# pierrepaleo/sift_pyocl

Hardware: AMD Instinct MI355X
Metric: SiftPlan.keypoints throughput, 4096x4096 fp32 (Mpix/s; keypoints/s in keypoints_per_s) (higher is better)
Workload: dtype f32

## Files before the change

### sift_pyocl_amd/csrc/k_pyramid.hpp

```cpp
#pragma once
#include <hip/hip_runtime.h>
#include <type_traits>
#include <stdint.h>
#include "k_xcd.hpp"

namespace siftk {

__device__ __forceinline__ uint32_t f2ord(float f) {
    uint32_t u = __float_as_uint(f);
    return (u & 0x80000000u) ? ~u : (u | 0x80000000u);
}
__device__ __forceinline__ float ord2f(uint32_t u) {
    return __uint_as_float((u & 0x80000000u) ? (u & 0x7fffffffu) : ~u);
}

__global__ void minmax_init(uint32_t *mm) { mm[0] = 0xffffffffu; mm[1] = 0u; }

__device__ __forceinline__ void minmax_reset_next(uint32_t *reset, int reset_words, int reset_ones) {
    if (reset && blockIdx.x == 0)
        for (int i = threadIdx.x; i < reset_words; i += blockDim.x) reset[i] = (i == reset_ones) ? 0xffffffffu : 0u;
}

__global__ __launch_bounds__(1024) void minmax_kernel(const float *__restrict__ img, int64_t n, uint32_t *mm, uint32_t *reset = nullptr,
                                                      int reset_words = 0, int reset_ones = -1) {
// ... 450 lines not shown
                        }                                                                                    \
                        const int done = (kk + 1) % N;                                                       \
                        const int y = ybase_ + kk;                                                           \
                        if (y >= ys && y < yend && !((BLUR_ABL & 8) && acc[done].x != 12345.678f)) {        \
                            if (vec_store) *reinterpret_cast<f32x2 *>(optr) = acc[done];                     \
                            else { if (gxo < W) optr[0] = acc[done].x; if (gxo + 1 < W) optr[1] = acc[done].y; } \
                            if (next0 && !(y & 1) && (y >> 1) < (H >> 1) && (gxo >> 1) < (W >> 1))           \
                                next0[(size_t)(y >> 1) * (W >> 1) + (gxo >> 1)] = acc[done].x;              \
                        }                                                                                    \
                        optr += W;                                                                           \
                    }                                                                                        \
                }                                                                                            \
            }                                                                                                \
        }                                                                                                    \
    }

    auto exists = [&](int blk, int sub) { return blk < nblocks - 1 || (blk == nblocks - 1 && sub < last_subs); };
    if (role == 1) {
        prefetch(0, 0, SS::pairs(0));
        stage(sbase, SS::pairs(0));
        if (S > 1) { if (exists(0, 1 % S)) prefetch(0, 1 % S, SS::pairs(1 % S)); }
        else if (exists(1, 0)) prefetch(1, 0, SS::pairs(0));
    }
    __syncthreads();
    int g = 0;
    const int total_steps = (nblocks - 1) * S + last_subs;
    int prio_level = -1;
    auto set_prio = [&](int step) {
        if (!prio) return;
        const int q = (step * 4) / total_steps;
        if (q == prio_level) return;
        prio_level = q;
        if (q <= 0) __builtin_amdgcn_s_setprio(3);
        else if (q == 1) __builtin_amdgcn_s_setprio(2);
        else if (q == 2) __builtin_amdgcn_s_setprio(1);
        else __builtin_amdgcn_s_setprio(0);
    };
    set_prio(0);
    if (role == 0) {
        for (int blk = 0; blk < nblocks; blk++) {
#pragma unroll
            for (int sub = 0; sub < S; sub++) {
                if (blk == nblocks - 1 && sub >= last_subs) break;
                hpass(sbase + (g % 3) * BUF, SS::pairs(sub));
                __syncthreads();
                g++;
                set_prio(g);
            }
        }
        return;
    }
    for (int blk = 0; blk < nblocks; blk++) {
#pragma unroll
        for (int sub = 0; sub < S; sub++) {
            if (blk == nblocks - 1 && sub >= last_subs) break;
            if (g > 0) {
                float *prev = sbase + ((g + 2) % 3) * BUF;
                if (sub == 0) { VPASS(prev, blk - 1, S - 1) } else { VPASS(prev, blk, (sub + S - 1) % S) }
            }
            const int sub1 = (sub + 1) % S, blk1 = blk + (sub + 1) / S;
            if (exists(blk1, sub1)) {
                float *nxt = sbase + ((g + 1) % 3) * BUF;
                stage(nxt, SS::pairs(sub1));
                const int sub2 = (sub + 2) % S;
                const int blk2 = blk + (sub + 2) / S;
                if (exists(blk2, sub2)) prefetch(blk2, sub2, SS::pairs(sub2));
            }
            __syncthreads();
            g++;
            set_prio(g);
        }
    }
    {
        float *prev = sbase + ((g + 2) % 3) * BUF;
        if (last_subs >= S) { VPASS(prev, nblocks - 1, S - 1) }
        if constexpr (S > 1) { if (last_subs == 1) { VPASS(prev, nblocks - 1, 0) } }
        if constexpr (S > 2) { if (last_subs == 2) { VPASS(prev, nblocks - 1, 1) } }
        if constexpr (S > 3) { if (last_subs == 3) { VPASS(prev, nblocks - 1, 2) } }
    }
#undef VPASS
}


__global__ void blur_generic_pass(const float *__restrict__ in, float *__restrict__ out, int W, int H,
                                  const float *__restrict__ taps, int n, int vertical,
                                  const uint32_t *__restrict__ mm, int norm) {
    const int x = blockIdx.x * blockDim.x + threadIdx.x, y = blockIdx.y;
    if (x >= W || y >= H) return;
    const int c = (n & 1) ? n / 2 : n / 2 - 1;
    float mn = 0.f, range = 1.f;
    if (norm) { mn = ord2f(mm[0]); range = ord2f(mm[1]) - mn; }
    float acc = 0.f;
    for (int j = 0; j < n; j++) {
        float v;
        if (vertical) v = in[(size_t)reflect_index(y - c + j, H) * W + x];
        else v = in[(size_t)y * W + reflect_index(x - c + j, W)];
        if (norm) v = 255.0f * (v - mn) / range;
        acc = acc + v * taps[n - 1 - j];
    }
    out[(size_t)y * W + x] = acc;
}

__global__ __launch_bounds__(256) void shrink_kernel(const float *__restrict__ in, float *__restrict__ out, int LW, int SW, int SH) {
    const int x = (blockIdx.x * 64 + (threadIdx.x & 63)) * 4;
    const int y0 = (blockIdx.y * 4 + (threadIdx.x >> 6)) * 2;
    if (x >= SW) return;
    const bool vec_in = (LW & 1) == 0 && x + 3 < SW;
    const bool vec_out = (SW & 3) == 0;
#pragma unroll
    for (int r = 0; r < 2; r++) {
        const int y = y0 + r;
        if (y >= SH) break;
        const float *src = in + (size_t)(2 * y) * LW + 2 * x;
        float *dst = out + (size_t)y * SW + x;
        if (vec_in) {
            const float4 a = *reinterpret_cast<const float4 *>(src), b = *reinterpret_cast<const float4 *>(src + 4);
            if (vec_out) *reinterpret_cast<float4 *>(dst) = make_float4(a.x, a.z, b.x, b.z);
            else { dst[0] = a.x; dst[1] = a.z; dst[2] = b.x; dst[3] = b.z; }
        } else {
            for (int k = 0; k < 4 && x + k < SW; k++) dst[k] = src[2 * k];
        }
    }
}
inline dim3 shrink_grid(int SW, int SH) { return dim3((unsigned)((SW + 255) / 256), (unsigned)((SH + 7) / 8)); }

template <int DT = 0>
__global__ void normalize_kernel(const void *__restrict__ in, float *__restrict__ out, int64_t n,
                                 const uint32_t *__restrict__ mm) {
    const float mn = ord2f(mm[0]), range = ord2f(mm[1]) - mn;
    const int64_t stride = (int64_t)gridDim.x * blockDim.x;
    for (int64_t i = (int64_t)blockIdx.x * blockDim.x + threadIdx.x; i < n; i += stride)
        out[i] = 255.0f * (load_px<DT>(in, (size_t)i) - mn) / range;
}

}
```

### sift_pyocl_amd/csrc/siftmi.hip

```cpp
#include <hip/hip_runtime.h>
#include <hip/hip_ext.h>

#include <cmath>
#include <cstdarg>
#include <cstdio>
#include <cstdlib>
#include <cstring>
#include <algorithm>
#include <chrono>
#include <mutex>
#include <new>
#include <unordered_map>
#include <string>
#include <vector>

#include "../../include/siftmi.h"
#include "k_extrema.hpp"
#include "k_keypoint.hpp"
#include "k_descriptor.hpp"
#include "k_align.hpp"
#include "k_match.hpp"
#include "k_pyramid.hpp"
#include "k_tail.hpp"
#include "siftmath.hpp"

using namespace siftk;

static_assert(sizeof(siftmi_keypoint) == 144, "siftmi_keypoint must be 144 bytes");

namespace {

thread_local std::string g_err;

#ifndef SIFT_SYNC_EVENT
#define SIFT_SYNC_EVENT (hipEventDisableTiming | hipEventDisableSystemFence)
#endif
#define SIFTMI_ETAILRETRY (-100)
#define SIFTMI_EGROW (-101)
int fail(int code, const char *fmt, ...) {
    char buf[512];
    va_list ap;
    va_start(ap, fmt);
    vsnprintf(buf, sizeof buf, fmt, ap);
    va_end(ap);
    g_err = buf;
    return code;
}

#define HIPCHK(expr)                                                                           \
    do {                                                                                       \
        hipError_t e_ = (expr);                                                                \
        if (e_ != hipSuccess)                                                                  \
            return fail(e_ == hipErrorOutOfMemory ? SIFTMI_ENOMEM : SIFTMI_EDEVICE, "%s: %s", #expr, \
                        hipGetErrorString(e_));                                                \
    } while (0)

int nextpower(int n) { int p = 1; while (p < n) p <<= 1; return p; }

int gaussian_taps(float sigma, int size, float *out) {
    if (size < 1 || size > 1024) return fail(SIFTMI_EINVAL, "gaussian size %d out of range", size);
    int P = nextpower(size);
    if (P < 2) P = 2;
    std::vector<float> g((size_t)P, 0.0f), sum((size_t)P, 0.0f);
    const float norm = sqrtf(2.0f * SM_PI_F);
    for (int i = 0; i < size; i++) {
        const float x = ((float)i - ((float)size - 1.0f) / 2.0f) / sigma;
        const float y = siftmath::expf_(-x * x / 2.0f);
        g[(size_t)i] = y / sigma / norm;
        sum[(size_t)i] = g[(size_t)i];
    }
    for (int stride = 512; stride >= 2; stride >>= 1)
        if (size > stride)
            for (int i = 0; i < stride && i + stride < P; i++) sum[(size_t)i] += sum[(size_t)(i + stride)];
    sum[0] += sum[1];
    for (int i = 0; i < size; i++) out[i] = g[(size_t)i] / sum[0];
    return SIFTMI_OK;
}

int kernel_size(double sigma) {
    int size = (int)std::ceil(2.0 * 4.0 * sigma + 1.0);
    if (size % 2 == 0) size += 1;
    return size;
}

struct Taps { int n = 0; float t[64] = {0}; float *dev = nullptr; };

#define SIFT_LDS_PAD_MAX 65536

struct Options {
    int fused_convert = 1;
    int overlap = 1;
    int march = 1;
    int march_wgs = 0;
    int xcd_map = 1;
    int march_prio = 1;
    int ori_blocks = 4096, ori_pad = 0;
    int desc_blocks = 960, desc_pad = 0;
    int desc_small_blocks = 576;
    int desc_dense_blocks = 960;
    int desc_stream = 0;
    int maps = 2, maps_density = 200;
    int maps_blocks = 8192;
    int mm_blocks = 256;
    int mm_threads = 1024;
    int desc_team = 2048;
    int fork = 2;
    int split = 0;
    int early_chain = 2;
    int desc_early_blocks = 704;
    int fused_refine = 1;
    int fused_shrink = 1;
    int ori_team = 1024;
    int desc_dynamic = 1;
    int tail_pixels = SIFT_TAIL_MAX_PIXELS;
    int tail = 1;
    int ext_rows = 0;
    int ext_strips = 2000;
    int ori_small_blocks = 608;
    int spin = 1;
    int host_timing = 0;
    int tail_fault = 0;
};
const Options g_default_options{};

struct Event { std::string label; hipEvent_t a = nullptr, b = nullptr; bool is_blur = false; double pixels = 0; int octave = -1; int launches = 1; };

size_t dtype_size(int dt) {
    switch (dt) {
        case SIFTMI_F32: return 4; case SIFTMI_U8: return 1; case SIFTMI_U16: return 2; case SIFTMI_U32: return 4;
        case SIFTMI_U64: return 8; case SIFTMI_I32: return 4; case SIFTMI_I64: return 8; case SIFTMI_F64: return 8;
        case SIFTMI_RGB8: return 3;
    }
    return 0;
}

}

struct GroupLists {
    float4 *kp = nullptr;  int *kp_aux = nullptr;  int64_t cap_kp = 0;
    float4 *okp = nullptr; int *oaux = nullptr;    int64_t cap_out = 0;
    float4 *cand = nullptr; int64_t cap_cand = 0;
};

struct siftmi_plan {
    void *chain = nullptr;
    int device = 0;
    hipStream_t stream = nullptr;
    int H = 0, W = 0, dtype = 0;
    siftmi_params par{};
    Options opt;
    int profile = 0;
    int n_oct = 0;
    std::vector<int> ow, oh;
    int64_t kpsize = 0;
    int64_t bytes = 0;
    float *planes = nullptr;
    std::vector<size_t> oct_off;
    float *tmp = nullptr;
    float *tmp_later = nullptr;
    float *tmp_below = nullptr;
    hipStream_t stream2 = nullptr;
    hipStream_t stream3 = nullptr;
    int64_t acc_calls = 0, acc_b0_launches = 0;
    double acc_total_ms = 0, acc_b0_ms = 0, acc_b0_pixels = 0;
    hipEvent_t ev_early = nullptr;
    hipEvent_t ev_p3 = nullptr;
    std::vector<hipEvent_t> ev_pyr;
    bool overlap = true;
    float *plane(int o, int s) const { return planes + oct_off[(size_t)o] + (size_t)s * (size_t)ow[(size_t)o] * (size_t)oh[(size_t)o]; }
    void *raw = nullptr;
    int raw_dtype = -1;
    Counters *cnt_pair = nullptr;
    int cnt_parity = 0;
    hipStream_t fin = nullptr;
    int last_group0 = 0;
// ... 25 lines not shown
    int64_t cap_rec = 0;
    bool in_flight = false;
    bool records_cut = false;
    int64_t grows = 0;
    int64_t tail_timeouts = 0;
    KpRecord *host_out = nullptr;
    int host_cap = 0;
    bool desc_rows = true;
    Taps taps[6];
    bool have_init = false;
    std::vector<Event> events;
    size_t n_events = 0;
    hipEvent_t ev_first = nullptr, ev_last[3] = {nullptr, nullptr, nullptr};
    float last_min = 0, last_max = 0;
    int64_t last_count = 0;
    int last_overflow = 0;
    std::vector<void *> allocs;

    template <class T> int alloc(T **p, size_t nbytes) {
        void *q = nullptr;
        hipError_t e = hipMalloc(&q, nbytes ? nbytes : 16);
        if (e != hipSuccess) return fail(SIFTMI_ENOMEM, "hipMalloc(%zu bytes): %s", nbytes, hipGetErrorString(e));
        allocs.push_back(q);
        bytes += (int64_t)nbytes;
        *p = (T *)q;
        return SIFTMI_OK;
    }
    template <class T> int regrow(T **p, size_t old_bytes, size_t new_bytes) {
        void *q = nullptr;
        hipError_t e = hipMalloc(&q, new_bytes ? new_bytes : 16);
        if (e != hipSuccess) return fail(SIFTMI_ENOMEM, "hipMalloc(%zu bytes): %s", new_bytes, hipGetErrorString(e));
        if (*p) { (void)hipFree(*p); bytes -= (int64_t)old_bytes; }
        bytes += (int64_t)new_bytes;
        *p = (T *)q;
        return SIFTMI_OK;
    }
};

namespace {

int compute_schedule(siftmi_plan *p) {
    const double init_sigma = p->par.init_sigma;
    p->have_init = false;
    p->desc_rows = (int)(1.414 * 3.0 * init_sigma * std::pow(2.0, 1.5) * 2.5 + 0.5) + 2 <= SIFT_DESC_MAXRAD;
    const double cur_sigma = p->par.double_im_size ? 1.0 : 0.5;
    if (init_sigma > cur_sigma) {
        const double s = std::sqrt(init_sigma * init_sigma - cur_sigma * cur_sigma);
        p->taps[5].n = kernel_size(s);
        if (p->taps[5].n > 64) return fail(SIFTMI_EINVAL, "init_sigma %g needs %d taps (> 64)", init_sigma, p->taps[5].n);
        int rc = gaussian_taps((float)s, p->taps[5].n, p->taps[5].t);
        if (rc) return rc;
        p->have_init = true;
    }
    const double ratio = std::pow(2.0, 1.0 / 3.0);
    double prev = init_sigma;
    for (int s = 0; s < 5; s++) {
        const double inc = prev * std::sqrt(ratio * ratio - 1.0);
        p->taps[s].n = kernel_size(inc);
        if (p->taps[s].n > 64) return fail(SIFTMI_EINVAL, "sigma %g needs %d taps (> 64)", inc, p->taps[s].n);
        int rc = gaussian_taps((float)inc, p->taps[s].n, p->taps[s].t);
        if (rc) return rc;
        prev *= ratio;
    }
    for (int s = 0; s < 6; s++) {
        if (!p->taps[s].dev) { int rc = p->alloc(&p->taps[s].dev, 64 * sizeof(float)); if (rc) return rc; }
        HIPCHK(hipMemcpy(p->taps[s].dev, p->taps[s].t, 64 * sizeof(float), hipMemcpyHostToDevice));
    }
    return SIFTMI_OK;
}

template <typename K, typename... A>
inline void launch_ev(hipEvent_t stop, K kernel, dim3 grid, dim3 block, size_t lds, hipStream_t st, A... args) {
    if (stop) hipExtLaunchKernelGGL(kernel, grid, block, (uint32_t)lds, st, nullptr, stop, 0u, args...);
    else hipLaunchKernelGGL(kernel, grid, block, lds, st, args...);
}

template <int N, bool NORM, int DT, int TX, int TY, int VR>
void launch_blur_geom(hipStream_t st, const void *in, float *out, int W, int H, const TapsArg<N> &ta, const uint32_t *mm, float *half, hipEvent_t stop = nullptr) {
    using G = BlurGeom<N, TX, TY>;
    dim3 grid((unsigned)((W + TX - 1) / TX), (unsigned)((H + TY - 1) / TY));
    launch_ev(stop, blur_hv_kernel<N, NORM, DT, TX, TY, VR>, grid, dim3(256), (size_t)G::LDS_BYTES, st, in, out, W, H, ta, mm, half);
}

template <int N, bool NORM, int DT = 0>
void launch_blur_t(const Options &opt, hipStream_t st, const void *in, float *out, int W, int H, const float *taps, const uint32_t *mm, float *half = nullptr, hipEvent_t stop = nullptr) {
    TapsArg<N> ta;
    for (int i = 0; i < N; i++) ta.t[i] = taps[i];
    (void)opt;
    launch_blur_geom<N, NORM, DT, 32, 16, 4>(st, in, out, W, H, ta, mm, half, stop);
}

template <int N, bool NORM, int S, int DT = 0>
void launch_team(const Options &opt, hipStream_t st, const void *in, float *out, int W, int H, const float *taps, const uint32_t *mm, int wgs, float *half, hipEvent_t stop) {
    using G = March2Geom<N, 128, S>;
    using SS = SubSplit<N, S>;
    TapsArg<N> ta;
    for (int i = 0; i < N; i++) ta.t[i] = taps[i];
    if (opt.march_wgs > 0) wgs = opt.march_wgs;
    const int gx = (W + G::TX - 1) / G::TX;
    int gy = wgs / gx;
    if (gy < 1) gy = 1;
    if (gy > H) gy = H;
    int rows_out = (H + gy - 1) / gy;
    if (rows_out < 2 * N + 1) rows_out = 2 * N + 1;
    gy = (H + rows_out - 1) / rows_out;
    auto covered = [](int b, int m) { int r = b * N; for (int q = 0; q < m; q++) r += SS::rows(q); return r; };
    const int need = rows_out + N - 1;
    const int b = need / N;
    int m = 0;
    while (covered(b, m) < need) m++;
    const int nblocks = b + (m > 0 ? 1 : 0), last_subs = m > 0 ? m : S;
    dim3 grid((unsigned)gx, (unsigned)gy);
    const int prio = (opt.march_prio == 2 || (opt.march_prio == 1 && gx * gy >= 704)) ? 1 : 0;
    launch_ev(stop, blur_team_kernel<N, NORM, S, DT>, grid, dim3(256), (size_t)3 * G::LDS_BYTES, st, in, out, W, H, nblocks, last_subs,
              rows_out, ta, mm, half, opt.xcd_map, prio);
}

template <int N, bool NORM, int DT = 0>
bool launch_march_t(const Options &opt, hipStream_t st, const void *in, float *out, int W, int H, const float *taps, const uint32_t *mm, float *half = nullptr, hipEvent_t stop = nullptr) {
    constexpr int S = (N <= 15) ? 2 : (N <= 21 ? 3 : 4);
    launch_team<N, NORM, S, DT>(opt, st, in, out, W, H, taps, mm, N >= 27 ? 768 : 1024, half, stop);
    return half != nullptr;
}

inline bool march_plane(int W, int H) { return W >= 1024 && H >= 512 && (int64_t)W * H >= 1400 * 1400; }

template <bool NORM>
int launch_blur_tiled(const Options &opt, hipStream_t st, const float *in, float *out, int W, int H, const Taps &t, const uint32_t *mm, float *half = nullptr, hipEvent_t stop = nullptr) {
    bool symmetric = true;
    for (int i = 0; i < t.n / 2; i++) symmetric = symmetric && (memcmp(&t.t[i], &t.t[t.n - 1 - i], 4) == 0);
    if constexpr (NORM) {
        if (t.n != 15) return 0;
        if (march_plane(W, H) && symmetric && opt.march) return launch_march_t<15, NORM>(opt, st, in, out, W, H, t.t, mm, half, stop) ? 2 : 1;
        launch_blur_t<15, NORM>(opt, st, in, out, W, H, t.t, mm, half, stop);
        return half ? 2 : 1;
    } else {
    if (march_plane(W, H) && symmetric && opt.march) {
        switch (t.n) {
            case 11: return launch_march_t<11, NORM>(opt, st, in, out, W, H, t.t, mm, half, stop) ? 2 : 1;
            case 15: return launch_march_t<15, NORM>(opt, st, in, out, W, H, t.t, mm, half, stop) ? 2 : 1;
            case 17: return launch_march_t<17, NORM>(opt, st, in, out, W, H, t.t, mm, half, stop) ? 2 : 1;
            case 21: return launch_march_t<21, NORM>(opt, st, in, out, W, H, t.t, mm, half, stop) ? 2 : 1;
            case 27: return launch_march_t<27, NORM>(opt, st, in, out, W, H, t.t, mm, half, stop) ? 2 : 1;
            default: break;
        }
    }
    switch (t.n) {
        case 11: launch_blur_t<11, NORM>(opt, st, in, out, W, H, t.t, mm, half, stop); return half ? 2 : 1;
        case 15: launch_blur_t<15, NORM>(opt, st, in, out, W, H, t.t, mm, half, stop); return half ? 2 : 1;
        case 17: launch_blur_t<17, NORM>(opt, st, in, out, W, H, t.t, mm, half, stop); return half ? 2 : 1;
        case 21: launch_blur_t<21, NORM>(opt, st, in, out, W, H, t.t, mm, half, stop); return half ? 2 : 1;
        case 27: launch_blur_t<27, NORM>(opt, st, in, out, W, H, t.t, mm, half, stop); return half ? 2 : 1;
        default: return 0;
    }
    }
}

void launch_blur_generic(hipStream_t st, const float *in, float *out, float *tmp, int W, int H, const Taps &t,
                         const uint32_t *mm, bool norm) {
    dim3 grid((unsigned)((W + 255) / 256), (unsigned)H);
    hipLaunchKernelGGL(blur_generic_pass, grid, dim3(256), 0, st, in, tmp, W, H, t.dev, t.n, 0, mm, norm ? 1 : 0);
    hipLaunchKernelGGL(blur_generic_pass, grid, dim3(256), 0, st, (const float *)tmp, out, W, H, t.dev, t.n, 1, mm, 0);
}

bool launch_blur(siftmi_plan *p, const float *in, float *out, int W, int H, const Taps &t, bool norm, hipStream_t st = nullptr, float *half = nullptr,
                 hipEvent_t stop = nullptr) {
    if (!st) st = p->stream;
    Options opt = p->opt;
    if (opt.march_prio == 1 && st != p->stream) opt.march_prio = 2;
    const int r = norm ? launch_blur_tiled<true>(opt, st, in, out, W, H, t, p->mm, half, stop)
                       : launch_blur_tiled<false>(opt, st, in, out, W, H, t, p->mm, half, stop);
    if (!r) {
        float *tmp = (st == p->stream2 && p->tmp_below) ? p->tmp_below : ((st == p->stream3 && p->tmp_later) ? p->tmp_later : p->tmp);
        launch_blur_generic(st, in, out, tmp, W, H, t, p->mm, norm);
        if (stop) (void)hipEventRecord(stop, st);
    }
    return r == 2;
}

bool taps_symmetric(const Taps &t) {
    bool symmetric = true;
    for (int i = 0; i < t.n / 2; i++) symmetric = symmetric && (memcmp(&t.t[i], &t.t[t.n - 1 - i], 4) == 0);
    return symmetric;
}

template <int DT>
bool launch_init_blur_dt(const Options &opt, hipStream_t st, const void *in, float *out, int W, int H, const Taps &t, const uint32_t *mm) {
    if (t.n != 15) return false;
    if (march_plane(W, H) && taps_symmetric(t) && opt.march)
        launch_march_t<15, true, DT>(opt, st, in, out, W, H, t.t, mm);
    else
        launch_blur_t<15, true, DT>(opt, st, in, out, W, H, t.t, mm);
    return true;
}

#define SIFTMI_TYPED_DISPATCH(dt, CALL)                       \
    switch (dt) {                                             \
        case SIFTMI_U8: { constexpr int DT = 1; CALL; } break;   \
        case SIFTMI_U16: { constexpr int DT = 2; CALL; } break;  \
        case SIFTMI_U32: { constexpr int DT = 3; CALL; } break;  \
        case SIFTMI_U64: { constexpr int DT = 4; CALL; } break;  \
        case SIFTMI_I32: { constexpr int DT = 5; CALL; } break;  \
        case SIFTMI_I64: { constexpr int DT = 6; CALL; } break;  \
        case SIFTMI_RGB8: { constexpr int DT = 8; CALL; } break; \
        default: break;                                       \
    }

struct Scope {
    siftmi_plan *p; size_t idx = (size_t)-1; hipStream_t st;
    bool stop_bound = false;
    Scope(siftmi_plan *pl, const char *label, bool is_blur = false, double pixels = 0, hipStream_t s = nullptr, int octave = -1, bool record_start = true) : p(pl) {
        st = s ? s : p->stream;
        if (!p->profile || (p->profile == 1 && !(is_blur && octave == 0))) return;
        if (p->n_events == p->events.size()) {
            Event e;
            hipEventCreate(&e.a); hipEventCreate(&e.b);
            p->events.push_back(e);
        }
        idx = p->n_events++;
        Event &e = p->events[idx];
        e.label = label; e.is_blur = is_blur; e.pixels = pixels; e.octave = octave; e.launches = 1;
        if (record_start) hipEventRecord(e.a, st);
    }
    ~Scope() { if (idx != (size_t)-1 && !stop_bound) hipEventRecord(p->events[idx].b, st); }
};

int grid_for(int64_t n, int block, int max_blocks) {
    int64_t g = (n + block - 1) / block;
    if (g < 1) g = 1;
    if (g > max_blocks) g = max_blocks;
    return (int)g;
}

double contrast_threshold(const siftmi_params &par) { return 0.8 * (double)par.peak_thresh; }

OctaveTable octave_table(const siftmi_plan *p) {
    OctaveTable tab;
    memset(&tab, 0, sizeof tab);
    tab.base = p->planes;
    tab.gmap = p->gmap; tab.omap = p->omap;
    for (int o = 0; o < p->n_oct && o < SIFT_MAX_OCTAVES; o++) {
        tab.off[o] = (long long)p->oct_off[(size_t)o];
        tab.W[o] = p->ow[(size_t)o];
        tab.H[o] = p->oh[(size_t)o];
    }
    return tab;
}

int group_of(const siftmi_plan *p, int oct);
int cand_group_of(const siftmi_plan *p, int oct);
int64_t list_limit(const siftmi_plan *p, int what, int g) {
    const int64_t K = p->kpsize, O = std::max(1, p->n_oct);
    int64_t lim = what == 0 ? 3 * K : (what == 1 ? 3 * K * (g == 2 ? O : 1) : (what == 2 ? K * (g == 2 ? O : 1) : K * O));
    return std::min<int64_t>(lim, 0x7fffff00);
}

void drain_streams(siftmi_plan *p);
int grow_lists(siftmi_plan *p, const Counters *c, bool *grown = nullptr) {
    if (grown) *grown = false;
    bool drained = c == nullptr;
    auto quiesce = [&]() { if (!drained) { drain_streams(p); drained = true; } };
    const bool forks = p->n_oct > 2;
    auto want = [&](int64_t cap, int64_t need, int64_t limit) {
        if (need <= cap) return cap;
        if (!c) return std::min<int64_t>(limit, need);
        return std::min<int64_t>(limit, std::max<int64_t>(need + need / 4 + 64, cap));
    };
    for (int g = 0; g < SIFT_GROUPS; g++) {
        if (g == 1 && !forks) continue;
        GroupLists &G = p->grp[g];
        int64_t need_cand = p->kpsize, need_kp = p->kpsize, need_out = p->kpsize;
        if (c) {
            need_cand = 0;
            for (int o = 0; o < p->n_oct && o < SIFT_MAX_OCTAVES; o++) if (cand_group_of(p, o) == g) need_cand = std::max<int64_t>(need_cand, c->n_cand[o]);
            need_kp = c->g_kp[g]; need_out = c->g_out[g];
        }
// ... 1615 lines not shown
    }
    template <class T> T *as() { return (T *)p; }
};

int stage_begin(int device_id) {
    int ndev = siftmi_device_count();
    if (ndev < 1) return fail(SIFTMI_EDEVICE, "no HIP device available");
    if (device_id < 0 || device_id >= ndev) return fail(SIFTMI_EINVAL, "device %d out of range", device_id);
    HIPCHK(hipSetDevice(device_id));
    return SIFTMI_OK;
}

int stage_end() {
    HIPCHK(hipDeviceSynchronize());
    HIPCHK(hipGetLastError());
    return SIFTMI_OK;
}

}

extern "C" {

int siftmi_stage_gaussian_taps(float sigma, int32_t size, float *out) {
    if (!out) return fail(SIFTMI_EINVAL, "null argument");
    return gaussian_taps(sigma, size, out);
}

int32_t siftmi_stage_xcd_order(int32_t id, int32_t n) { return (n > 0 && id >= 0 && id < n) ? siftk::xcd_contiguous(id, n) : -1; }

int siftmi_stage_minmax_normalize(int32_t dev, const float *in, float *out, int32_t W, int32_t H, float *mn, float *mx) {
    int rc = stage_begin(dev); if (rc) return rc;
    const size_t N = (size_t)W * H;
    DevBuf a, b, mm;
    if ((rc = a.upload(in, N * 4)) || (rc = b.alloc(N * 4)) || (rc = mm.alloc(8))) return rc;
    hipLaunchKernelGGL(minmax_init, dim3(1), dim3(1), 0, 0, mm.as<uint32_t>());
    hipLaunchKernelGGL(minmax_kernel, dim3(grid_for((int64_t)N / 4, 256, 2048)), dim3(256), 0, 0, a.as<float>(), (int64_t)N, mm.as<uint32_t>());
    hipLaunchKernelGGL(normalize_kernel<0>, dim3(grid_for((int64_t)N, 256, 4096)), dim3(256), 0, 0, (const void *)a.as<float>(), b.as<float>(), (int64_t)N, (const uint32_t *)mm.as<uint32_t>());
    if ((rc = stage_end())) return rc;
    uint32_t h[2];
    HIPCHK(hipMemcpy(h, mm.p, 8, hipMemcpyDeviceToHost));
    auto dec = [](uint32_t u) { uint32_t v = (u & 0x80000000u) ? (u & 0x7fffffffu) : ~u; float f; memcpy(&f, &v, 4); return f; };
    if (mn) *mn = dec(h[0]);
    if (mx) *mx = dec(h[1]);
    if (out) HIPCHK(hipMemcpy(out, b.p, N * 4, hipMemcpyDeviceToHost));
    return SIFTMI_OK;
}

int siftmi_stage_blur(int32_t dev, const float *in, float *out, int32_t W, int32_t H, const float *taps, int32_t ntaps) {
    int rc = stage_begin(dev); if (rc) return rc;
    if (ntaps < 1 || ntaps > 64) return fail(SIFTMI_EINVAL, "ntaps must be in 1..64");
    const size_t N = (size_t)W * H;
    DevBuf a, b, t, dt;
    if ((rc = a.upload(in, N * 4)) || (rc = b.alloc(N * 4)) || (rc = t.alloc(N * 4))) return rc;
    Taps tp; tp.n = ntaps;
    for (int i = 0; i < ntaps; i++) tp.t[i] = taps[i];
    if ((rc = dt.upload(tp.t, sizeof tp.t))) return rc;
    tp.dev = dt.as<float>();
    if (!launch_blur_tiled<false>(g_default_options, 0, a.as<float>(), b.as<float>(), W, H, tp, nullptr))
        launch_blur_generic(0, a.as<float>(), b.as<float>(), t.as<float>(), W, H, tp, nullptr, false);
    if ((rc = stage_end())) return rc;
    HIPCHK(hipMemcpy(out, b.p, N * 4, hipMemcpyDeviceToHost));
    return SIFTMI_OK;
}

int siftmi_stage_blur_ex(int32_t dev, const void *in, int32_t in_dtype, float *out, int32_t W, int32_t H, const float *taps, int32_t ntaps,
                         int32_t norm, int32_t xcd_map, int32_t march_wgs, int32_t *kernel_used) {
    int rc = stage_begin(dev); if (rc) return rc;
    if (!in || !out || !taps || W < 1 || H < 1) return fail(SIFTMI_EINVAL, "null argument or empty plane");
    if (ntaps < 1 || ntaps > 64) return fail(SIFTMI_EINVAL, "ntaps must be in 1..64");
    const size_t esz = dtype_size(in_dtype);
    if (!esz || in_dtype == SIFTMI_F64) return fail(SIFTMI_EINVAL, "input format %d has no fused blur", in_dtype);
    if (in_dtype != SIFTMI_F32 && !(norm && ntaps == 15)) return fail(SIFTMI_EINVAL, "typed frames enter through the normalising 15-tap blur only");
    const size_t N = (size_t)W * H;
    DevBuf a, b, t, dt, mm;
    if ((rc = a.upload(in, N * esz)) || (rc = b.alloc(N * 4)) || (rc = t.alloc(N * 4)) || (rc = mm.alloc(8))) return rc;
    Taps tp; tp.n = ntaps;
    for (int i = 0; i < ntaps; i++) tp.t[i] = taps[i];
    if ((rc = dt.upload(tp.t, sizeof tp.t))) return rc;
    tp.dev = dt.as<float>();
    Options opt = g_default_options;
    opt.xcd_map = (xcd_map & 1) ? 1 : 0;
    opt.march_prio = (xcd_map & 2) ? 0 : 2;
    opt.march_wgs = march_wgs > 0 ? march_wgs : 0;
    uint32_t *mmp = mm.as<uint32_t>();
    if (norm) {
        hipLaunchKernelGGL(minmax_init, dim3(1), dim3(1), 0, 0, mmp);
        if (in_dtype == SIFTMI_F32) {
            hipLaunchKernelGGL(minmax_kernel, dim3(grid_for((int64_t)N / 4, 256, 2048)), dim3(256), 0, 0, a.as<float>(), (int64_t)N, mmp);
        } else {
            SIFTMI_TYPED_DISPATCH(in_dtype, hipLaunchKernelGGL(minmax_typed_kernel<DT>, dim3(grid_for((int64_t)N / TypedChunk<DT>::PX, 256, 256)), dim3(256), 0, 0,
                                                               (const void *)a.p, (int64_t)N, mmp));
        }
    }
    int used = 0;
    if (in_dtype != SIFTMI_F32) {
        bool ok = false;
        SIFTMI_TYPED_DISPATCH(in_dtype, ok = launch_init_blur_dt<DT>(opt, 0, (const void *)a.p, b.as<float>(), W, H, tp, mmp));
        if (!ok) return fail(SIFTMI_EINVAL, "no fused blur for input format %d", in_dtype);
        used = (march_plane(W, H) && taps_symmetric(tp) && opt.march) ? 2 : 1;
    } else {
        const int r = norm ? launch_blur_tiled<true>(opt, 0, a.as<float>(), b.as<float>(), W, H, tp, mmp)
                           : launch_blur_tiled<false>(opt, 0, a.as<float>(), b.as<float>(), W, H, tp, mmp);
        if (!r) launch_blur_generic(0, a.as<float>(), b.as<float>(), t.as<float>(), W, H, tp, mmp, norm != 0);
        else {
            bool marchable = false;
            for (int n : {11, 15, 17, 21, 27}) marchable = marchable || n == ntaps;
            used = (march_plane(W, H) && taps_symmetric(tp) && opt.march && marchable) ? 2 : 1;
        }
    }
    if ((rc = stage_end())) return rc;
    if (kernel_used) *kernel_used = used;
    HIPCHK(hipMemcpy(out, b.p, N * 4, hipMemcpyDeviceToHost));
    return SIFTMI_OK;
}

int siftmi_stage_dog(int32_t dev, const float *blur_a, const float *blur_b, float *out, int64_t n) {
    int rc = stage_begin(dev); if (rc) return rc;
    DevBuf a, b, o;
    if ((rc = a.upload(blur_a, (size_t)n * 4)) || (rc = b.upload(blur_b, (size_t)n * 4)) || (rc = o.alloc((size_t)n * 4))) return rc;
    hipLaunchKernelGGL(dog_kernel, dim3(grid_for(n, 256, 4096)), dim3(256), 0, 0, a.as<float>(), b.as<float>(), o.as<float>(), n);
    if ((rc = stage_end())) return rc;
    HIPCHK(hipMemcpy(out, o.p, (size_t)n * 4, hipMemcpyDeviceToHost));
    return SIFTMI_OK;
}

int siftmi_stage_local_maxmin(int32_t dev, const float *blurs, int32_t W, int32_t H, int32_t octsize,
                              const siftmi_params *par, float *out, int64_t capacity, int64_t *n_out) {
    int rc = stage_begin(dev); if (rc) return rc;
    if (!par || !n_out) return fail(SIFTMI_EINVAL, "null argument");
    const size_t N = (size_t)W * H;
    DevBuf b, c, cnt;
    if ((rc = b.upload(blurs, 6 * N * 4)) || (rc = c.alloc((size_t)capacity * 16)) || (rc = cnt.alloc(sizeof(Counters)))) return rc;
    HIPCHK(hipMemset(cnt.p, 0, sizeof(Counters)));
    BlurPlanes bp;
    for (int s = 0; s < 6; s++) bp.p[s] = b.as<float>() + (size_t)s * N;
    const int border = par->border_dist;
    if (W > 2 * border && H > 2 * border) {
        const int rows = extrema_strip_rows(W, H, border);
        const int nx = (W - 2 * border + 61) / 62, ny = (H - 2 * border + rows - 1) / rows;
        const float edth = (octsize <= 1) ? par->edge_thresh0 : par->edge_thresh;
        hipLaunchKernelGGL(extrema_kernel<false>, dim3((unsigned)((nx * ny + 3) / 4)), dim3(256), 0, 0, bp, W, H, border, rows,
                           contrast_threshold(*par), edth, c.as<float4>(), &cnt.as<Counters>()->n_cand[0], (int)capacity, RefineArgs{}, -1, -1, 1);
    }
    if ((rc = stage_end())) return rc;
    Counters hc;
    HIPCHK(hipMemcpy(&hc, cnt.p, sizeof hc, hipMemcpyDeviceToHost));
    int64_t n = hc.n_cand[0] < capacity ? hc.n_cand[0] : capacity;
    if (n > 0) HIPCHK(hipMemcpy(out, c.p, (size_t)n * 16, hipMemcpyDeviceToHost));
    *n_out = n;
    return SIFTMI_OK;
}

int siftmi_stage_interp(int32_t dev, const float *blurs, int32_t W, int32_t H, const float *cand, int64_t n,
                        const siftmi_params *par, float *out, int32_t *out_scale, int64_t *n_out) {
    int rc = stage_begin(dev); if (rc) return rc;
    if (!par || !n_out) return fail(SIFTMI_EINVAL, "null argument");
    const size_t N = (size_t)W * H;
    DevBuf b, c, k, ks, cnt;
    if ((rc = b.upload(blurs, 6 * N * 4)) || (rc = c.upload(cand, (size_t)n * 16)) || (rc = k.alloc((size_t)n * 16)) ||
        (rc = ks.alloc((size_t)n * 4)) || (rc = cnt.alloc(sizeof(Counters)))) return rc;
    Counters hc{};
    hc.n_cand[0] = (int)n;
    HIPCHK(hipMemcpy(cnt.p, &hc, sizeof hc, hipMemcpyHostToDevice));
    BlurPlanes bp;
    for (int s = 0; s < 6; s++) bp.p[s] = b.as<float>() + (size_t)s * N;
    Counters *dc = cnt.as<Counters>();
    hipLaunchKernelGGL(refine_kernel, dim3(grid_for(n, 256, 512)), dim3(256), 0, 0, bp, W, H, (const float4 *)c.as<float4>(),
                       (const int *)&dc->n_cand[0], (int)n, par->peak_thresh, (float)par->init_sigma, k.as<float4>(),
                       ks.as<int>(), &dc->g_kp[0], (int)n, 0, &dc->c_scale[0][0]);
    if ((rc = stage_end())) return rc;
    HIPCHK(hipMemcpy(&hc, cnt.p, sizeof hc, hipMemcpyDeviceToHost));
    const int64_t m = hc.g_kp[0];
    if (m > 0) {
        HIPCHK(hipMemcpy(out, k.p, (size_t)m * 16, hipMemcpyDeviceToHost));
        HIPCHK(hipMemcpy(out_scale, ks.p, (size_t)m * 4, hipMemcpyDeviceToHost));
    }
    *n_out = m;
    return SIFTMI_OK;
}

int siftmi_stage_compact(int32_t dev, const float *kps, int64_t n, int64_t start, int64_t end, float *out, int64_t *n_out) {
    int rc = stage_begin(dev); if (rc) return rc;
    if (!n_out || start < 0 || end < start || end > n) return fail(SIFTMI_EINVAL, "bad range");
    DevBuf a, o, cnt;
    if ((rc = a.upload(kps, (size_t)n * 16)) || (rc = o.alloc((size_t)n * 16)) || (rc = cnt.alloc(16))) return rc;
    HIPCHK(hipMemcpy(o.p, a.p, (size_t)start * 16, hipMemcpyDeviceToDevice));
    const int first = (int)start;
    HIPCHK(hipMemcpy(cnt.p, &first, 4, hipMemcpyHostToDevice));
    if (end > start)
        hipLaunchKernelGGL(compact_kernel, dim3(grid_for(end - start, 256, 1024)), dim3(256), 0, 0, (const float4 *)a.as<float4>(),
                           o.as<float4>(), cnt.as<int>(), (int)start, (int)end, (int)n);
// ... 142 lines not shown
```

Before: 21630.

## Add packed-pair tile blur kernel for mid-size pyramid planes

Adds a new separable Gaussian blur kernel that loads a tile into LDS with row pairs packed as float2. It runs the horizontal pass in place with a symmetric-tap folded register convolution, then runs the vertical pass over 8-row segments and writes float2 outputs plus an optional half-resolution copy. Launch dispatch now picks this kernel for symmetric taps on planes of at least 600x600 that are not handled by the march team kernel, choosing a taller tile for planes of a megapixel or more. The point is to cut LDS traffic and arithmetic in the smaller octave blurs. The trade-off is a larger halo per tile and a more complex LDS layout.

```diff
diff --git a/sift_pyocl_amd/csrc/k_pyramid.hpp b/sift_pyocl_amd/csrc/k_pyramid.hpp
--- a/sift_pyocl_amd/csrc/k_pyramid.hpp
+++ b/sift_pyocl_amd/csrc/k_pyramid.hpp
@@ -556,6 +556,124 @@
 }
 
 
+template <int N, int L, class RD> __device__ __forceinline__ void blur_segment(const float (&t)[N], RD rd, f32x2 (&acc)[L]) {
+#pragma unroll
+    for (int j = 0; j < L; j++) acc[j] = (f32x2){0.f, 0.f};
+#pragma unroll
+    for (int i = 0; i < L + N - 1; i++) {
+        const f32x2 x = rd(i);
+#pragma unroll
+        for (int k = 0; k <= (N - 1) / 2; k++) {
+            const int ya = i - k, yb = i - (N - 1 - k);
+            const bool na = ya >= 0 && ya < L, nb = k != N - 1 - k && yb >= 0 && yb < L;
+            if (!na && !nb) continue;
+            const f32x2 p = x * (f32x2){t[k], t[k]};
+            if (na) acc[ya] = acc[ya] + p;
+            if (nb) acc[yb] = acc[yb] + p;
+        }
+    }
+}
+
+template <int N, int TX, int TY> struct Tile2Geom {
+    static constexpr int C = N / 2;
+    static constexpr int L = 8, VR = 8;
+    static constexpr int ROWS = TY + N - 1, RP = ROWS / 2;
+    static constexpr int COLS = TX + N - 1;
+    static constexpr int PITCH = (COLS + 1) & ~1;
+    static constexpr int LDS_BYTES = RP * PITCH * 8;
+};
+
+template <int N, bool NORM, int DT = 0, int TX = 32, int TY = 64>
+__global__ __launch_bounds__(256) void blur_tile2_kernel(const void *__restrict__ in, float *__restrict__ out,
+                                                         int W, int H, TapsArg<N> taps,
+                                                         const uint32_t *__restrict__ mm,
+                                                         float *__restrict__ half) {
+    using G = Tile2Geom<N, TX, TY>;
+    static_assert(N & 1, "odd tap counts only");
+    static_assert(TY % G::VR == 0 && TX % G::L == 0 && 64 % (TX / G::L) == 0 && G::COLS <= 128, "tile shape");
+    extern __shared__ float4 smem4[];
+    float *s = reinterpret_cast<float *>(smem4);
+    const int tid = threadIdx.x, lane = tid & 63;
+    const int wave = __builtin_amdgcn_readfirstlane(tid >> 6);
+    const int x0 = blockIdx.x * TX, y0 = blockIdx.y * TY;
+
+    float mn = 0.f, range = 1.f;
+    if (NORM) { mn = ord2f(mm[0]); range = ord2f(mm[1]) - mn; }
+
+    {
+        const int c1 = lane + 64;
+        const bool has0 = lane < G::COLS, has1 = c1 < G::COLS;
+        const int gxa = reflect_index(x0 - G::C + lane, W), gxb = reflect_index(x0 - G::C + (has1 ? c1 : lane), W);
+        const int ytop = y0 - G::C;
+        const bool inside = ytop >= 0 && ytop + G::ROWS <= H;
+        auto fetch = [&](int gy, int gx) {
+            float v = load_px<DT>(in, (size_t)gy * W + gx);
+            if (NORM) v = 255.0f * (v - mn) / range;
+            return v;
+        };
+        f32x2 *s2 = reinterpret_cast<f32x2 *>(s);
+        if (inside) {
+#pragma unroll 2
+            for (int rp = wave; rp < G::RP; rp += 4) {
+                const int gy = ytop + 2 * rp;
+                if (has0) s2[rp * G::PITCH + lane] = (f32x2){fetch(gy, gxa), fetch(gy + 1, gxa)};
+                if (has1) s2[rp * G::PITCH + c1] = (f32x2){fetch(gy, gxb), fetch(gy + 1, gxb)};
+            }
+        } else {
+#pragma unroll 2
+            for (int rp = wave; rp < G::RP; rp += 4) {
+                const int gy0 = reflect_index(ytop + 2 * rp, H), gy1 = reflect_index(ytop + 2 * rp + 1, H);
+                if (has0) s2[rp * G::PITCH + lane] = (f32x2){fetch(gy0, gxa), fetch(gy1, gxa)};
+                if (has1) s2[rp * G::PITCH + c1] = (f32x2){fetch(gy0, gxb), fetch(gy1, gxb)};
+            }
+        }
+    }
+    __syncthreads();
+
+    constexpr int HT = TX / G::L;
+    for (int task = tid; task < G::RP * HT; task += 256) {
+        const int rp = task / HT, c0 = (task - rp * HT) * G::L;
+        float *rowp = s + (rp * G::PITCH + c0) * 2;
+        f32x2 acc[G::L];
+        blur_segment<N, G::L>(taps.t, [&](int i) { return *reinterpret_cast<const f32x2 *>(rowp + 2 * i); }, acc);
+        __builtin_amdgcn_wave_barrier();
+#pragma unroll
+        for (int j = 0; j < G::L; j += 2)
+            *reinterpret_cast<f32x4 *>(rowp + 2 * j) = (f32x4){acc[j].x, acc[j + 1].x, acc[j].y, acc[j + 1].y};
+    }
+    __syncthreads();
+
+    constexpr int CP = TX / 2;
+    for (int task = tid; task < CP * (TY / G::VR); task += 256) {
+        const int rg = task / CP, c = (task - rg * CP) * 2;
+        const int r0 = rg * G::VR;
+        const float *colp = s + ((r0 / 2) * G::PITCH + c) * 2;
+        f32x4 v;
+        f32x2 acc[G::VR];
+        blur_segment<N, G::VR>(taps.t, [&](int i) {
+            if (!(i & 1)) v = *reinterpret_cast<const f32x4 *>(colp + (i / 2) * G::PITCH * 2);
+            return (i & 1) ? v.zw : v.xy;
+        }, acc);
+        const int gx = x0 + c;
+        const bool vec = ((W & 1) == 0) && gx + 1 < W;
+#pragma unroll
+        for (int j = 0; j < G::VR; j++) {
+            const int gy = y0 + r0 + j;
+            if (gy < H) {
+                float *o = out + (size_t)gy * W + gx;
+                if (vec) *reinterpret_cast<f32x2 *>(o) = acc[j];
+                else {
+                    if (gx < W) o[0] = acc[j].x;
+                    if (gx + 1 < W) o[1] = acc[j].y;
+                }
+                if (half && !(gy & 1) && (gy >> 1) < (H >> 1) && (gx >> 1) < (W >> 1))
+                    half[(size_t)(gy >> 1) * (W >> 1) + (gx >> 1)] = acc[j].x;
+            }
+        }
+    }
+}
+
+
 __global__ void blur_generic_pass(const float *__restrict__ in, float *__restrict__ out, int W, int H,
                                   const float *__restrict__ taps, int n, int vertical,
                                   const uint32_t *__restrict__ mm, int norm) {
diff --git a/sift_pyocl_amd/csrc/siftmi.hip b/sift_pyocl_amd/csrc/siftmi.hip
--- a/sift_pyocl_amd/csrc/siftmi.hip
+++ b/sift_pyocl_amd/csrc/siftmi.hip
@@ -91,6 +91,7 @@
     int fused_convert = 1;
     int overlap = 1;
     int march = 1;
+    int small_blur = 2;
     int march_wgs = 0;
     int xcd_map = 1;
     int march_prio = 1;
@@ -282,12 +283,33 @@
     launch_ev(stop, blur_hv_kernel<N, NORM, DT, TX, TY, VR>, grid, dim3(256), (size_t)G::LDS_BYTES, st, in, out, W, H, ta, mm, half);
 }
 
+template <int N, bool NORM, int DT, int TX, int TY>
+void launch_tile2(hipStream_t st, const void *in, float *out, int W, int H, const TapsArg<N> &ta, const uint32_t *mm, float *half, hipEvent_t stop) {
+    using G = Tile2Geom<N, TX, TY>;
+    dim3 grid((unsigned)((W + TX - 1) / TX), (unsigned)((H + TY - 1) / TY));
+    launch_ev(stop, blur_tile2_kernel<N, NORM, DT, TX, TY>, grid, dim3(256), (size_t)G::LDS_BYTES, st, in, out, W, H, ta, mm, half);
+}
+
+enum BlurForm { BLUR_NONE = 0, BLUR_TILE = 1, BLUR_TEAM = 2, BLUR_TILE2 = 3 };
+
+constexpr int64_t TILE2_MIN_PIXELS = 600 * 600;
+constexpr int64_t TILE2_TALL_PIXELS = 1024 * 1024;
+inline bool tile2_plane(const Options &opt, int W, int H, bool symmetric) {
+    return symmetric && (opt.small_blur == 1 || (opt.small_blur == 2 && (int64_t)W * H >= TILE2_MIN_PIXELS));
+}
+
 template <int N, bool NORM, int DT = 0>
-void launch_blur_t(const Options &opt, hipStream_t st, const void *in, float *out, int W, int H, const float *taps, const uint32_t *mm, float *half = nullptr, hipEvent_t stop = nullptr) {
+BlurForm launch_blur_t(const Options &opt, hipStream_t st, const void *in, float *out, int W, int H, const float *taps, bool symmetric,
+                       const uint32_t *mm, float *half = nullptr, hipEvent_t stop = nullptr) {
     TapsArg<N> ta;
     for (int i = 0; i < N; i++) ta.t[i] = taps[i];
-    (void)opt;
+    if (tile2_plane(opt, W, H, symmetric)) {
+        if ((int64_t)W * H >= TILE2_TALL_PIXELS) launch_tile2<N, NORM, DT, 32, 64>(st, in, out, W, H, ta, mm, half, stop);
+        else launch_tile2<N, NORM, DT, 32, 32>(st, in, out, W, H, ta, mm, half, stop);
+        return BLUR_TILE2;
+    }
     launch_blur_geom<N, NORM, DT, 32, 16, 4>(st, in, out, W, H, ta, mm, half, stop);
+    return BLUR_TILE;
 }
 
 template <int N, bool NORM, int S, int DT = 0>
@@ -325,33 +347,37 @@
 
 inline bool march_plane(int W, int H) { return W >= 1024 && H >= 512 && (int64_t)W * H >= 1400 * 1400; }
 
-template <bool NORM>
-int launch_blur_tiled(const Options &opt, hipStream_t st, const float *in, float *out, int W, int H, const Taps &t, const uint32_t *mm, float *half = nullptr, hipEvent_t stop = nullptr) {
+bool taps_symmetric(const Taps &t) {
     bool symmetric = true;
     for (int i = 0; i < t.n / 2; i++) symmetric = symmetric && (memcmp(&t.t[i], &t.t[t.n - 1 - i], 4) == 0);
+    return symmetric;
+}
+
+template <bool NORM>
+BlurForm launch_blur_tiled(const Options &opt, hipStream_t st, const float *in, float *out, int W, int H, const Taps &t, const uint32_t *mm, float *half = nullptr, hipEvent_t stop = nullptr) {
+    const bool symmetric = taps_symmetric(t);
     if constexpr (NORM) {
-        if (t.n != 15) return 0;
-        if (march_plane(W, H) && symmetric && opt.march) return launch_march_t<15, NORM>(opt, st, in, out, W, H, t.t, mm, half, stop) ? 2 : 1;
-        launch_blur_t<15, NORM>(opt, st, in, out, W, H, t.t, mm, half, stop);
-        return half ? 2 : 1;
+        if (t.n != 15) return BLUR_NONE;
+        if (march_plane(W, H) && symmetric && opt.march) { launch_march_t<15, NORM>(opt, st, in, out, W, H, t.t, mm, half, stop); return BLUR_TEAM; }
+        return launch_blur_t<15, NORM>(opt, st, in, out, W, H, t.t, symmetric, mm, half, stop);
     } else {
     if (march_plane(W, H) && symmetric && opt.march) {
         switch (t.n) {
-            case 11: return launch_march_t<11, NORM>(opt, st, in, out, W, H, t.t, mm, half, stop) ? 2 : 1;
-            case 15: return launch_march_t<15, NORM>(opt, st, in, out, W, H, t.t, mm, half, stop) ? 2 : 1;
-            case 17: return launch_march_t<17, NORM>(opt, st, in, out, W, H, t.t, mm, half, stop) ? 2 : 1;
-            case 21: return launch_march_t<21, NORM>(opt, st, in, out, W, H, t.t, mm, half, stop) ? 2 : 1;
-            case 27: return launch_march_t<27, NORM>(opt, st, in, out, W, H, t.t, mm, half, stop) ? 2 : 1;
+            case 11: launch_march_t<11, NORM>(opt, st, in, out, W, H, t.t, mm, half, stop); return BLUR_TEAM;
+            case 15: launch_march_t<15, NORM>(opt, st, in, out, W, H, t.t, mm, half, stop); return BLUR_TEAM;
+            case 17: launch_march_t<17, NORM>(opt, st, in, out, W, H, t.t, mm, half, stop); return BLUR_TEAM;
+            case 21: launch_march_t<21, NORM>(opt, st, in, out, W, H, t.t, mm, half, stop); return BLUR_TEAM;
+            case 27: launch_march_t<27, NORM>(opt, st, in, out, W, H, t.t, mm, half, stop); return BLUR_TEAM;
             default: break;
         }
     }
     switch (t.n) {
-        case 11: launch_blur_t<11, NORM>(opt, st, in, out, W, H, t.t, mm, half, stop); return half ? 2 : 1;
-        case 15: launch_blur_t<15, NORM>(opt, st, in, out, W, H, t.t, mm, half, stop); return half ? 2 : 1;
-        case 17: launch_blur_t<17, NORM>(opt, st, in, out, W, H, t.t, mm, half, stop); return half ? 2 : 1;
-        case 21: launch_blur_t<21, NORM>(opt, st, in, out, W, H, t.t, mm, half, stop); return half ? 2 : 1;
-        case 27: launch_blur_t<27, NORM>(opt, st, in, out, W, H, t.t, mm, half, stop); return half ? 2 : 1;
-        default: return 0;
+        case 11: return launch_blur_t<11, NORM>(opt, st, in, out, W, H, t.t, symmetric, mm, half, stop);
+        case 15: return launch_blur_t<15, NORM>(opt, st, in, out, W, H, t.t, symmetric, mm, half, stop);
+        case 17: return launch_blur_t<17, NORM>(opt, st, in, out, W, H, t.t, symmetric, mm, half, stop);
+        case 21: return launch_blur_t<21, NORM>(opt, st, in, out, W, H, t.t, symmetric, mm, half, stop);
+        case 27: return launch_blur_t<27, NORM>(opt, st, in, out, W, H, t.t, symmetric, mm, half, stop);
+        default: return BLUR_NONE;
     }
     }
 }
@@ -368,30 +394,22 @@
     if (!st) st = p->stream;
     Options opt = p->opt;
     if (opt.march_prio == 1 && st != p->stream) opt.march_prio = 2;
-    const int r = norm ? launch_blur_tiled<true>(opt, st, in, out, W, H, t, p->mm, half, stop)
-                       : launch_blur_tiled<false>(opt, st, in, out, W, H, t, p->mm, half, stop);
-    if (!r) {
+    const BlurForm r = norm ? launch_blur_tiled<true>(opt, st, in, out, W, H, t, p->mm, half, stop)
+                            : launch_blur_tiled<false>(opt, st, in, out, W, H, t, p->mm, half, stop);
+    if (r == BLUR_NONE) {
         float *tmp = (st == p->stream2 && p->tmp_below) ? p->tmp_below : ((st == p->stream3 && p->tmp_later) ? p->tmp_later : p->tmp);
         launch_blur_generic(st, in, out, tmp, W, H, t, p->mm, norm);
         if (stop) (void)hipEventRecord(stop, st);
     }
-    return r == 2;
-}
-
-bool taps_symmetric(const Taps &t) {
-    bool symmetric = true;
-    for (int i = 0; i < t.n / 2; i++) symmetric = symmetric && (memcmp(&t.t[i], &t.t[t.n - 1 - i], 4) == 0);
-    return symmetric;
+    return r != BLUR_NONE && half;
 }
 
 template <int DT>
-bool launch_init_blur_dt(const Options &opt, hipStream_t st, const void *in, float *out, int W, int H, const Taps &t, const uint32_t *mm) {
-    if (t.n != 15) return false;
-    if (march_plane(W, H) && taps_symmetric(t) && opt.march)
-        launch_march_t<15, true, DT>(opt, st, in, out, W, H, t.t, mm);
-    else
-        launch_blur_t<15, true, DT>(opt, st, in, out, W, H, t.t, mm);
-    return true;
+BlurForm launch_init_blur_dt(const Options &opt, hipStream_t st, const void *in, float *out, int W, int H, const Taps &t, const uint32_t *mm) {
+    if (t.n != 15) return BLUR_NONE;
+    const bool symmetric = taps_symmetric(t);
+    if (march_plane(W, H) && symmetric && opt.march) { launch_march_t<15, true, DT>(opt, st, in, out, W, H, t.t, mm); return BLUR_TEAM; }
+    return launch_blur_t<15, true, DT>(opt, st, in, out, W, H, t.t, symmetric, mm);
 }
 
 #define SIFTMI_TYPED_DISPATCH(dt, CALL)                       \
@@ -2173,6 +2191,7 @@
     opt.xcd_map = (xcd_map & 1) ? 1 : 0;
     opt.march_prio = (xcd_map & 2) ? 0 : 2;
     opt.march_wgs = march_wgs > 0 ? march_wgs : 0;
+    if ((xcd_map >> 2) & 3) opt.small_blur = ((xcd_map >> 2) & 3) - 1;
     uint32_t *mmp = mm.as<uint32_t>();
     if (norm) {
         hipLaunchKernelGGL(minmax_init, dim3(1), dim3(1), 0, 0, mmp);
@@ -2183,21 +2202,14 @@
                                                                (const void *)a.p, (int64_t)N, mmp));
         }
     }
-    int used = 0;
+    BlurForm used = BLUR_NONE;
     if (in_dtype != SIFTMI_F32) {
-        bool ok = false;
-        SIFTMI_TYPED_DISPATCH(in_dtype, ok = launch_init_blur_dt<DT>(opt, 0, (const void *)a.p, b.as<float>(), W, H, tp, mmp));
-        if (!ok) return fail(SIFTMI_EINVAL, "no fused blur for input format %d", in_dtype);
-        used = (march_plane(W, H) && taps_symmetric(tp) && opt.march) ? 2 : 1;
+        SIFTMI_TYPED_DISPATCH(in_dtype, used = launch_init_blur_dt<DT>(opt, 0, (const void *)a.p, b.as<float>(), W, H, tp, mmp));
+        if (used == BLUR_NONE) return fail(SIFTMI_EINVAL, "no fused blur for input format %d", in_dtype);
     } else {
-        const int r = norm ? launch_blur_tiled<true>(opt, 0, a.as<float>(), b.as<float>(), W, H, tp, mmp)
-                           : launch_blur_tiled<false>(opt, 0, a.as<float>(), b.as<float>(), W, H, tp, mmp);
-        if (!r) launch_blur_generic(0, a.as<float>(), b.as<float>(), t.as<float>(), W, H, tp, mmp, norm != 0);
-        else {
-            bool marchable = false;
-            for (int n : {11, 15, 17, 21, 27}) marchable = marchable || n == ntaps;
-            used = (march_plane(W, H) && taps_symmetric(tp) && opt.march && marchable) ? 2 : 1;
-        }
+        used = norm ? launch_blur_tiled<true>(opt, 0, a.as<float>(), b.as<float>(), W, H, tp, mmp)
+                    : launch_blur_tiled<false>(opt, 0, a.as<float>(), b.as<float>(), W, H, tp, mmp);
+        if (used == BLUR_NONE) launch_blur_generic(0, a.as<float>(), b.as<float>(), t.as<float>(), W, H, tp, mmp, norm != 0);
     }
     if ((rc = stage_end())) return rc;
     if (kernel_used) *kernel_used = used;
```

New measurement: 22050, median of 6. 1.9% higher.
